# AI4quantum/twisteRL

Hardware: AMD Instinct MI355X
Metric: env-steps/s (whole node) Puzzle-15 PPO rollout (higher is better)
Workload: dtype f32; 1 GPU; Puzzle-15 PPO rollout + GAE + merge: 262144 envs/GPU, difficulty 128 (<= 257 records/episode), twists {identity, transpose}, BasicPolicy 256->512->256->4|1, gamma=lambda=0.995, torch-default-init weights seed 0; total_envs=262144, parallelism=episodes sharded x1

## Files before the change

### twisterl_amd/csrc/tw_engine.hpp

```cpp
#pragma once
#include <type_traits>
#include "tw_common.hpp"
#include "tw_engine_generic.hpp"
#include <cstdlib>

namespace tw {

typedef float f32x16 __attribute__((ext_vector_type(16)));
typedef float f32x4 __attribute__((ext_vector_type(4)));
typedef float f32x2 __attribute__((ext_vector_type(2)));
typedef __attribute__((address_space(3))) const float lds_cfloat;

constexpr int EPW = 32;


__device__ __forceinline__ float relu1(float x)
{
    float y;
    asm("v_max_f32 %0, 0, %1\n\ts_nop 1" : "=v"(y) : "v"(x));
    return y;
}
__device__ __forceinline__ float relu_lim(float x, float lim)
{
    float y;
    asm("v_max_f32 %0, %1, %2\n\ts_nop 1" : "=v"(y) : "s"(lim), "v"(x));
    return y;
}

__device__ __forceinline__ f32x2 pk_add(f32x2 a, f32x2 b)
{
    f32x2 r;
    r[0] = a[0] + b[0]; r[1] = a[1] + b[1];
    return r;
}

__device__ __forceinline__ float relu_lim_v(float x, float lim)
{
    float y;
    asm("v_max_f32 %0, %1, %2" : "=v"(y) : "s"(lim), "v"(x));
    return y;
}

__device__ __forceinline__ int gumbel_argmax4_halves(const float l[4], const u32x4 w, bool upper)
{
// ... 21 lines not shown

template <int NT>
__host__ __device__ inline size_t engine3_lds_floats(int obs_size)
{
    return (size_t)3 * R3_KC * Tiles<NT>::NQ * 128 + (size_t)3 * R3_TSLOT + (size_t)NT * 32 * 10 + 8 +
           (size_t)MAX_LDS_PERMS * ((obs_size + 3) / 4 + 1) + (size_t)NT * 32 * 5;
}

template <int NT, int NC, int NW_ = 8>
struct Engine3 {
    static constexpr int NW = NW_, KC = R3_KC, THREADS = 64 * NW_, EPB = NW * EPW, LSTR = R3_LSTR;
    static constexpr int NQ     = Tiles<NT>::NQ;
    static constexpr int WSLOT  = KC * NQ * 128;
    static constexpr int WPIECE = WSLOT / 256;
    static constexpr int TPIECE = ((NC * NC + 2) * R3_LSTR * 4 + 1023) / 1024;
    static_assert(TPIECE * 256 <= R3_TSLOT, "table chunk larger than its slot");
    static constexpr int NPIECE = WPIECE + TPIECE;
    static constexpr int NOPS   = (NPIECE + NW - 1) / NW;
    static constexpr int M      = 4 * NT;
    static constexpr bool SPLIT = false;

    __host__ __device__ static size_t lds_floats(int obs_size) { return engine3_lds_floats<NT>(obs_size); }
    __host__ __device__ static size_t lds_floats(const PolicyDev &p) { return lds_floats(p.obs_size); }
    __device__ __forceinline__ bool primary() const { return true; }
    __device__ __forceinline__ int  ep_lane() const { return wave * EPW + j; }
    __device__ __forceinline__ bool owns_lane() const { return true; }

    PolicyDev pol;
    int tid, lane, wave, j, h;
    uint32_t voff;
    int bias_row, zero_row, n_chunks;
    float emb_lim, common_lim;
    float *lds_w, *lds_t, *lds_b1, *lds_wh, *lds_bh, *lds_wn;
    const uint8_t *perm_obs, *perm_act;

    static_assert(WPIECE % NW == 0, "W1 pieces per chunk must be a multiple of the wave count");
    const uint8_t *dsrc_w, *dsrc_t;
    uint32_t ddst_w, ddst_t;
    __device__ __forceinline__ void stream_op(int chunk, int slot, int op)
    {
        if (NW * op < WPIECE) {
            const uint8_t *src = dsrc_w + (size_t)chunk * (WSLOT * 4) + (size_t)op * (NW * 1024);
            const uint32_t dst = ddst_w + (uint32_t)slot * (WSLOT * 4) + (uint32_t)op * (NW * 1024);
            TW_GLDS16(voff, dst, src);
        } else {
            const int T0 = NW * op - WPIECE;
            uint32_t tp = (uint32_t)wave + (uint32_t)T0;
            if (T0 + NW - 1 >= TPIECE) tp = tp < (uint32_t)TPIECE ? tp : (uint32_t)TPIECE - 1u;
            const uint8_t *src = dsrc_t + (size_t)chunk * (R3_TSLOT * 4) + (size_t)tp * 1024;
            const uint32_t dst = ddst_t + (uint32_t)slot * (R3_TSLOT * 4) + tp * 1024u;
            TW_GLDS16(voff, dst, src);
        }
    }

    __device__ __forceinline__ void begin1(const PolicyDev &p, float *lds)
    {
        pol = p;
        tid  = threadIdx.x;
        lane = tid & 63;
        wave = __builtin_amdgcn_readfirstlane(tid >> 6);
        j = lane & 31; h = lane >> 5;
        voff = (uint32_t)lane * 16u;
        bias_row = pol.obs_size; zero_row = pol.obs_size + 1;
        n_chunks = pol.emb / KC;
        emb_lim = pol.emb_relu ? 0.0f : -__builtin_inff();
        common_lim = pol.common_relu ? 0.0f : -__builtin_inff();
        lds_w  = lds;
        lds_t  = lds + 3 * WSLOT;
        lds_b1 = lds_t + 3 * R3_TSLOT;
        lds_wh = lds_b1 + NT * 32;
        lds_bh = lds_wh + NT * 32 * 9;
        dsrc_w = reinterpret_cast<const uint8_t *>(pol.w1p) + (size_t)wave * 1024;
        dsrc_t = reinterpret_cast<const uint8_t *>(pol.t_img16);
        ddst_w = __builtin_amdgcn_readfirstlane((unsigned)(uintptr_t)(__attribute__((address_space(3))) float *)lds_w) + (uint32_t)wave * 1024u;
        ddst_t = __builtin_amdgcn_readfirstlane((unsigned)(uintptr_t)(__attribute__((address_space(3))) float *)lds_t);
        for (int i = tid; i < NT * 32; i += THREADS) lds_b1[(i & 1) * (NT * 16) + (i >> 1)] = pol.b1[i];
        for (int i = tid; i < NT * 32 * 8; i += THREADS) {
            const int n = i >> 3, c = i & 7;
            lds_wh[(c * 2 + (n & 1)) * (NT * 16) + (n >> 1)] = pol.wh8[i];
        }
        for (int i = tid; i < NT * 32; i += THREADS) lds_wh[8 * 2 * (NT * 16) + i] = 0.0f;
        if (tid < 8) lds_bh[tid] = pol.bh8[tid];
        lds_wn = lds_bh + 8 + MAX_LDS_PERMS * ((pol.obs_size + 3) / 4 + 1);
        for (int i = tid; i < NT * 32 * 5; i += THREADS) {
            const int c = i / (NT * 32), n = i - c * (NT * 32);
            lds_wn[i] = pol.wh8[n * 8 + c];
        }
        perm_obs = pol.obs_perms; perm_act = pol.act_perms;
        if (pol.n_perms > 0 && pol.n_perms <= MAX_LDS_PERMS) {
            uint8_t *po = reinterpret_cast<uint8_t *>(lds_bh + 8);
            uint8_t *pa = po + MAX_LDS_PERMS * ((pol.obs_size + 3) / 4) * 4;
            for (int i = tid; i < pol.n_perms * pol.obs_size; i += THREADS) po[i] = pol.obs_perms[i];
            for (int i = tid; i < pol.n_perms * 4; i += THREADS) pa[i] = pol.act_perms[i];
            perm_obs = po; perm_act = pa;
        }
#pragma unroll
        for (int op = 0; op < NOPS; ++op) { stream_op(0, 0, op); stream_op(n_chunks > 1 ? 1 : 0, 1, op); }
    }
    __device__ __forceinline__ void begin2() { asm volatile("s_waitcnt vmcnt(0)" ::: "memory"); }
    __device__ __forceinline__ void end() { asm volatile("s_waitcnt vmcnt(0)" ::: "memory"); }

    __device__ __forceinline__ void rows_of(uint64_t board, int n_cells, int perm, int (&rowoff)[NC]) const
    {
#pragma unroll
        for (int i = 0; i < NC; ++i) {
            int row = zero_row;
            if (i < n_cells) {
                const int id = i * n_cells + (int)nib(board, i);
                row = perm >= 0 ? (int)perm_obs[perm * pol.obs_size + id] : id;
            }
            rowoff[i] = row * LSTR + h * (KC / 2);
        }
    }

    __device__ __forceinline__ void act_perm(int perm, float (&lg)[4]) const
    {
        if (perm < 0) return;
        const float l0 = lg[0], l1 = lg[1], l2 = lg[2], l3 = lg[3];
#pragma unroll
        for (int i = 0; i < 4; ++i) {
            const int src = perm_act[perm * 4 + i];
            lg[i] = src == 0 ? l0 : (src == 1 ? l1 : (src == 2 ? l2 : l3));
        }
    }

    __device__ __forceinline__ void finish_b(f32x4 &b) const
    {
        float x0 = b[0], x1 = b[1], x2 = b[2], x3 = b[3];
        asm("v_max_f32 %0, %4, %0\n\tv_max_f32 %1, %4, %1\n\tv_max_f32 %2, %4, %2\n\tv_max_f32 %3, %4, %3"
            : "+v"(x0), "+v"(x1), "+v"(x2), "+v"(x3) : "s"(emb_lim));
        b[0] = x0; b[1] = x1; b[2] = x2; b[3] = x3;
    }

    template <bool HAVE_NEXT_GATHER, bool LAST, bool CROSS>
    __device__ __forceinline__ void group(f32x16 (&acc)[NT], f32x4 (&aw)[NQ], const f32x4 bq, const float *w_base, int kp0,
                                          const float *wn_base, lds_cfloat *const (&ga)[NC + 1], int goff, f32x4 &bnext,
                                          int s_chunk, int s_slot, int op0, int op1)
    {
        constexpr int LAT = M >= 16 ? 4 : 1;
        auto rd_slot  = [](int q) constexpr { return M >= 16 ? (q * (M - 6)) / (NC + 1) : 0; };
        auto add_slot = [&](int q) constexpr { int v = rd_slot(q) + LAT; return v > M - 1 ? M - 1 : v; };
        f32x4 rd[NC + 1];
        f32x2 nlo, nhi;
#pragma unroll
        for (int m = 0; m < M; ++m) {
            const int u = m / NT, r = m % NT;
            acc[r] = __builtin_amdgcn_mfma_f32_32x32x2f32(aw[r / 4][r % 4], bq[u], acc[r], 0, 0, 0);
            __builtin_amdgcn_sched_barrier(0);
            if (r % 4 == 3 || r == NT - 1) {
                if (u < 3 || !LAST) aw[r / 4] = *reinterpret_cast<const f32x4 *>(w_base + ((kp0 + u + 1) * 2 * NQ + r / 4) * 128);
                else if (CROSS) aw[r / 4] = *reinterpret_cast<const f32x4 *>(wn_base + (r / 4) * 128);
            }
            {
                if constexpr (NW == 8) {
// ... 508 lines not shown
        this->tid = threadIdx.x; this->lane = this->tid & 63; this->wave = __builtin_amdgcn_readfirstlane(this->tid >> 6);
        this->j = this->lane & 15; this->h = this->lane >> 4;
        this->n_chunks = this->pol.emb / KC;
        np = (this->n_chunks + 1) / 2;
        n2 = (np + 1) / 2 * 2;
        __builtin_amdgcn_s_barrier();
    }
    __device__ __forceinline__ void idle_forward() const
    {
        for (int i = 0; i < n2 + 3; ++i) __builtin_amdgcn_s_barrier();
    }
    template <int SLOT, int OP = 0>
    __device__ __forceinline__ void stream_pair() const
    {
        if constexpr (OP < NOPS) { stream<SLOT, OP>(); stream_pair<SLOT, OP + 1>(); }
    }
    __device__ __forceinline__ int real_pair(int v) const { return v < np ? v : (v < n2 ? 0 : v - n2); }
    __device__ __forceinline__ void set_pointers()
    {
        stp  = this->dsrc_t + (size_t)real_pair(sv) * (2 * R3_TSLOT * 4);
        aoff = real_pair(av) * (2 * WSLOT);
    }
    __device__ __forceinline__ void advance()
    {
        ++sv; ++av; stp += 2 * R3_TSLOT * 4; aoff += 2 * WSLOT;
        if (sv == np || sv == n2) stp = this->dsrc_t;
        if (av == np || av == n2) aoff = 0;
        if (sv == n2) sv = 0;
        if (av == n2) av = 0;
    }

    __device__ __forceinline__ void rows_of(uint64_t board, int n_cells, int perm, int (&rowoff)[NC]) const
    {
#pragma unroll
        for (int i = 0; i < NC; ++i) {
            int row = this->zero_row;
            if (i < n_cells) {
                const int id = i * n_cells + (int)nib(board, i);
                row = perm >= 0 ? (int)this->perm_obs[perm * this->pol.obs_size + id] : id;
            }
            rowoff[i] = row * R3_LSTR;
        }
    }

    template <bool EB = false>
    __device__ __forceinline__ void forward(const int (&rowoff)[NC], float (&lg)[4], float &value)
    {
        typedef __attribute__((address_space(3))) const f32x4 lds_cf4;
        const int jj = this->j, kq = this->h, wave = this->wave;
        f32x4v acc[TPW];
#pragma unroll
        for (int t = 0; t < TPW; ++t) acc[t] = f32x4v{0.0f, 0.0f, 0.0f, 0.0f};

        lds_cfloat *gb = (lds_cfloat *)tbase + ((kq & 1) * 8 + 2 * wave + (kq >> 1));
        lds_cfloat *ga[NC + 1];
        ga[0] = gb + this->bias_row * R3_LSTR;
#pragma unroll
        for (int c = 0; c < NC; ++c) ga[c + 1] = gb + rowoff[c];

        float *xb = lds_x + 256;
        float gr[2][NC + 1];
        auto gather_finish = [&](int buf) {
#pragma unroll
            for (int hf = 0; hf < 2; ++hf) {
                float sm = gr[hf][0];
#pragma unroll
                for (int c = 1; c <= NC; ++c) sm = sm + gr[hf][c];
                xb[(buf * 64 + this->lane) * 8 + hf * 4 + wave] = relu_lim_v(sm, this->emb_lim);
            }
        };

        int par = 0;
        auto step = [&](auto pc, int p) {
            constexpr int P = decltype(pc)::value, Q = P ^ 1;
            constexpr int M = 8 * TPW;
// ... 102 lines not shown
```

### twisterl_amd/csrc/tw_engine16.hpp

```cpp
#pragma once
#include "tw_engine.hpp"

#include <type_traits>

namespace tw {

typedef _Float16 h16x8 __attribute__((ext_vector_type(8)));
typedef _Float16 h16x2 __attribute__((ext_vector_type(2)));
typedef __attribute__((address_space(3))) const uint8_t lds_cu8;

constexpr int E16_MAXP   = 4;
constexpr int E16_MAX_KT = 32;

template <int NHT, int NC>
__host__ __device__ constexpr size_t engine16_lds_bytes()
{
    return 160 + (size_t)(E16_MAXP + 1) * (16 + 256) + 32 + (size_t)2 * (E16_MAXP + 1) * 256 + 64 + (size_t)NHT * 128 + (size_t)E16_MAX_KT * 128 +
           (size_t)NHT * 2048 + (size_t)NC * 1024 + (size_t)3 * ((NC + 2 * NHT + 3) / 4) * 4096;
}

template <int NHT, int NC>
struct Engine16 {
    static constexpr int NW = 4, THREADS = 256, EPB = 256, D = 3;
    static constexpr int SP     = NC + 2 * NHT;
    static constexpr int NOPS   = (SP + NW - 1) / NW;
    static constexpr int SBYTES = NOPS * NW * 1024;
    static constexpr float OUT_SCALE = 1.0f;
    static constexpr bool SPLIT_RANGE = false;
    static constexpr uint32_t O_OH = 0, O_SRC = 160, O_VMAP = O_SRC + (E16_MAXP + 1) * 16, O_ACT = O_VMAP + (E16_MAXP + 1) * 256,
                              O_OHB = O_ACT + 32, O_BH = O_OHB + 2 * (E16_MAXP + 1) * 256, O_B1 = O_BH + 64, O_EBIAS = O_B1 + NHT * 128, O_HEAD = O_EBIAS + E16_MAX_KT * 128,
                              O_T0 = O_HEAD + NHT * 2048, O_RING = O_T0 + NC * 1024;
    static_assert(O_RING + 3 * SBYTES == engine16_lds_bytes<NHT, NC>(), "LDS map");

    struct Pipe { h16x8 a[D], x0[D], x1[D]; f32x16 eb; };
    struct OneHots { uint32_t a0[NC], a1[NC]; };

    PolicyDev pol;
    int tid, lane, wave, j, hh, n_kt, rp;
    TW_STAMP_VARS(st[8] = {});
    uint8_t *lg_;
    uint32_t lds_u32, voff;
    lds_cu8 *L;
// ... 34 lines not shown
        for (int i = tid; i < np1 * 16; i += THREADS) lds[O_SRC + i] = pol.srcmap16[i];
        for (int i = tid; i < np1 * 256; i += THREADS) lds[O_VMAP + i] = pol.vmap16[i];
        for (int i = tid; i < 2 * np1 * 256; i += THREADS) {
            const int h2 = i / (np1 * 256), r = i - h2 * (np1 * 256);
            const uint32_t pos = (uint32_t)pol.vmap16[r] ^ ((uint32_t)h2 << 3);
            lds[O_OHB + h2 * ((E16_MAXP + 1) * 256) + r] = (uint8_t)((pos < 8u ? pos : 8u) * 16u);
        }
        if (tid < 4) lds[O_ACT + tid] = (uint8_t)tid;
        for (int i = tid; i < pol.n_perms * 4; i += THREADS) lds[O_ACT + 4 + i] = pol.act_perms[i];
        for (int i = tid; i < n_kt * 32; i += THREADS) reinterpret_cast<float *>(lds + O_EBIAS)[i] = pol.ebias16[i];
#pragma unroll
        for (int op = 0; op < NOPS; ++op) { stream_op(stage_ptr(0), slot_m0(0), op); stream_op(stage_ptr(n_kt > 1 ? 1 : 0), slot_m0(1), op); }
        rp = 0;
    }
    __device__ __forceinline__ void begin2() { asm volatile("s_waitcnt vmcnt(0)" ::: "memory"); }
    __device__ __forceinline__ void end() { asm volatile("s_waitcnt vmcnt(0)" ::: "memory"); }

    __device__ __forceinline__ void onehots(uint64_t board, int perm, uint32_t (&w)[NC]) const
    {
        static_assert(O_OH == 0, "the byte table holds LDS addresses");
        const int pi = perm + 1;
        typedef uint32_t u32v4 __attribute__((ext_vector_type(4)));
        const u32v4 sr = *(const __attribute__((address_space(3))) u32v4 *)(L + O_SRC + pi * 16);
        const uint32_t srw[4] = {sr[0], sr[1], sr[2], sr[3]};
        const uint32_t tb = O_OHB + (uint32_t)(hh * (E16_MAXP + 1) + pi) * 256u;
#pragma unroll
        for (int c = 0; c < NC; ++c) {
            const uint32_t src = (srw[c >> 2] >> (8 * (c & 3))) & 0xffu;
            const uint32_t v   = nib(board, (int)src);
            w[c] = L[tb + c * 16 + v];
        }
    }

    __device__ __forceinline__ void act_perm(int perm, float (&lg)[4]) const
    {
        typedef __attribute__((address_space(3))) const uint32_t lu1;
        const uint32_t ap = *(const lu1 *)(L + O_ACT + (perm + 1) * 4);
        const float l0 = lg[0], l1 = lg[1], l2 = lg[2], l3 = lg[3];
#pragma unroll
        for (int i = 0; i < 4; ++i) {
            const uint32_t src = (ap >> (8 * i)) & 0xffu;
            lg[i] = src == 0 ? l0 : (src == 1 ? l1 : (src == 2 ? l2 : l3));
        }
    }

    __device__ __forceinline__ f32x16 ld16(uint32_t off) const
    {
        typedef __attribute__((address_space(3))) const f32x4 lf4;
        const lf4 *p = (const lf4 *)(L + off);
        const f32x4 a = p[0], b = p[1], c = p[2], d = p[3];
        f32x16 r;
#pragma unroll
        for (int i = 0; i < 4; ++i) { r[i] = a[i]; r[4 + i] = b[i]; r[8 + i] = c[i]; r[12 + i] = d[i]; }
        return r;
    }
    __device__ __forceinline__ h16x8 ld8(uint32_t off) const
    {
        return *(const __attribute__((address_space(3))) h16x8 *)(L + off);
    }
    static __device__ __forceinline__ void mfma_v(f32x16 &d, const h16x8 a, const h16x8 b, bool first, const f32x16 &c0)
    {
        if (first) asm volatile("v_mfma_f32_32x32x16_f16 %0, %1, %2, %3" : "=&v"(d) : "v"(a), "v"(b), "v"(c0));
        else       asm volatile("v_mfma_f32_32x32x16_f16 %0, %1, %2, %0" : "+v"(d) : "v"(a), "v"(b));
    }
    template <bool BIAS>
    static __device__ __forceinline__ void cvt_unit(const f32x16 &e, const f32x16 &bias, int m, int q, h16x2 lim, h16x8 &dst)
// ... 208 lines not shown
```

### twisterl_amd/csrc/tw_engine16x2.hpp

```cpp
#pragma once
#include "tw_engine16.hpp"

#include <utility>

namespace tw {

template <int NHT, int NC>
__host__ __device__ constexpr int engineS_pieces() { return (NC + 2 * NHT > 4 * NHT) ? NC + 2 * NHT : 4 * NHT; }
template <int NHT, int NC>
__host__ __device__ constexpr size_t engineS_lds_bytes()
{
    return 160 + (size_t)(E16_MAXP + 1) * (16 + 256) + 32 + (size_t)2 * (E16_MAXP + 1) * 256 + 64 + (size_t)NHT * 128 +
           (size_t)E16_MAX_KT * 128 + (size_t)2 * NC * 1024 + (size_t)3 * ((engineS_pieces<NHT, NC>() + 3) / 4) * 4096;
}

template <int NHT, int NC>
struct EngineS {
    static constexpr int NW = 4, THREADS = 256, EPB = 256, D = 3;
    static constexpr int NM0    = 2 * NHT;
    static constexpr int SP     = engineS_pieces<NHT, NC>();
    static constexpr int NOPS   = (SP + NW - 1) / NW;
    static constexpr int SBYTES = NOPS * NW * 1024;
    static constexpr float OUT_SCALE = 1.0f / 4096.0f;
    static constexpr bool SPLIT_RANGE = true;
// ... 47 lines not shown
        for (int i = tid; i < np1 * 16; i += THREADS) lds[O_SRC + i] = pol.srcmap16[i];
        for (int i = tid; i < np1 * 256; i += THREADS) lds[O_VMAP + i] = pol.vmap16[i];
        for (int i = tid; i < 2 * np1 * 256; i += THREADS) {
            const int h2 = i / (np1 * 256), r = i - h2 * (np1 * 256);
            const uint32_t pos = (uint32_t)pol.vmap16[r] ^ ((uint32_t)h2 << 3);
            lds[O_OHB + h2 * ((E16_MAXP + 1) * 256) + r] = (uint8_t)((pos < 8u ? pos : 8u) * 16u);
        }
        if (tid < 4) lds[O_ACT + tid] = (uint8_t)tid;
        for (int i = tid; i < pol.n_perms * 4; i += THREADS) lds[O_ACT + 4 + i] = pol.act_perms[i];
        for (int i = tid; i < n_kt * 32; i += THREADS) reinterpret_cast<float *>(lds + O_EBIAS)[i] = pol.ebias16[i] * 16.0f;
#pragma unroll
        for (int op = 0; op < NOPS; ++op) { stream_op(stage_ptr(0), slot_m0(0), op); stream_op(stage_ptr(1), slot_m0(1), op); }
        rp = 0;
    }
    __device__ __forceinline__ void begin2() { asm volatile("s_waitcnt vmcnt(0)" ::: "memory"); }
    __device__ __forceinline__ void end() { asm volatile("s_waitcnt vmcnt(0)" ::: "memory"); }

    __device__ __forceinline__ void onehots(uint64_t board, int perm, uint32_t (&w)[(NC + 3) / 4]) const
    {
        static_assert(O_OH == 0, "the byte table holds LDS addresses");
        const int pi = perm + 1;
        typedef uint32_t u32v4 __attribute__((ext_vector_type(4)));
        const u32v4 sr = *(const __attribute__((address_space(3))) u32v4 *)(L + O_SRC + pi * 16);
        const uint32_t srw[4] = {sr[0], sr[1], sr[2], sr[3]};
        const uint32_t tb = O_OHB + (uint32_t)(hh * (E16_MAXP + 1) + pi) * 256u;
#pragma unroll
        for (int q = 0; q < (NC + 3) / 4; ++q) w[q] = 0u;
#pragma unroll
        for (int c = 0; c < NC; ++c) {
            const uint32_t src = (srw[c >> 2] >> (8 * (c & 3))) & 0xffu;
            w[c >> 2] |= (uint32_t)L[tb + c * 16 + nib(board, (int)src)] << (8 * (c & 3));
        }
    }
    __device__ __forceinline__ h16x8 ldoh(const uint32_t (&w)[(NC + 3) / 4], int c) const
    {
        return ld8(O_OH + ((w[c >> 2] >> (8 * (c & 3))) & 0xffu));
    }
    __device__ __forceinline__ void act_perm(int perm, float (&lg)[4]) const
    {
        typedef __attribute__((address_space(3))) const uint32_t lu1;
        const uint32_t ap = *(const lu1 *)(L + O_ACT + (perm + 1) * 4);
        const float l0 = lg[0], l1 = lg[1], l2 = lg[2], l3 = lg[3];
#pragma unroll
        for (int i = 0; i < 4; ++i) {
            const uint32_t src = (ap >> (8 * i)) & 0xffu;
            lg[i] = src == 0 ? l0 : (src == 1 ? l1 : (src == 2 ? l2 : l3));
        }
    }
    __device__ __forceinline__ f32x16 ld16(uint32_t off) const
    {
        typedef __attribute__((address_space(3))) const f32x4 lf4;
        const lf4 *p = (const lf4 *)(L + off);
        const f32x4 a = p[0], b = p[1], c = p[2], d = p[3];
        f32x16 r;
#pragma unroll
        for (int i = 0; i < 4; ++i) { r[i] = a[i]; r[4 + i] = b[i]; r[8 + i] = c[i]; r[12 + i] = d[i]; }
        return r;
    }
    __device__ __forceinline__ h16x8 ld8(uint32_t off) const { return *(const __attribute__((address_space(3))) h16x8 *)(L + off); }
    static __device__ __forceinline__ void mfma_v(f32x16 &d, const h16x8 a, const h16x8 b, bool first, const f32x16 &c0)
    {
        if (first) asm volatile("v_mfma_f32_32x32x16_f16 %0, %1, %2, %3" : "=&v"(d) : "v"(a), "v"(b), "v"(c0));
        else       asm volatile("v_mfma_f32_32x32x16_f16 %0, %1, %2, %0" : "+v"(d) : "v"(a), "v"(b));
    }
    static __device__ __forceinline__ void split_unit(const f32x16 &e, int m, int q, float lim, h16x8 &hi, h16x8 &lo)
    {
// ... 228 lines not shown
```

### twisterl_amd/csrc/tw_rollout.hip

```cpp
#include "tw_engine.hpp"

#include <cstdlib>
#include <cstring>

namespace tw {

__global__ void __launch_bounds__(256) init_boards_kernel(const PuzzleConsts env, uint64_t seed, uint64_t episode_offset, uint64_t n, uint64_t *out, uint4 *entries)
{
    const uint64_t i = (uint64_t)blockIdx.x * 256 + threadIdx.x;
    if (i >= n) return;
    PuzzleLane st;
    puzzle_reset(st, env, seed, episode_offset + i);
    if (out) out[i] = st.board;
    if (entries) entries[i] = make_uint4((uint32_t)st.board, (uint32_t)(st.board >> 32), (uint32_t)i, 0u);
}

int launch_init_boards(const PuzzleConsts &env, uint64_t seed, uint64_t episode_offset, uint64_t n, uint64_t *out, hipStream_t s, uint4 *entries)
{
    if (n == 0) return TW_OK;
    hipLaunchKernelGGL(init_boards_kernel, dim3((unsigned)((n + 255) / 256)), dim3(256), 0, s, env, seed, episode_offset, n, out, entries);
    TW_HIP(hipGetLastError());
    return TW_OK;
}

// ... 115 lines not shown
TW_STAMP_ARRAY(g_gen_stamps, 8);

template <int NT, int NC, int NW = 8, bool PERSIST = false>
__global__ void __launch_bounds__((Geom<NT, NC, NW>::WAVES * 64), ((NW == 8 || NW == -65) ? 2 : 1)) rollout_f32_kernel(const RolloutArgs a)
{
    using Eng = typename Geom<NT, NC, NW>::Eng;
    extern __shared__ __attribute__((aligned(16))) float lds[];
    Eng eng;
    eng.begin1(a.pol, lds);

    const PuzzleConsts env = a.env;
    const int j = eng.j, h = eng.h;
    const uint64_t e_first = (uint64_t)blockIdx.x * Eng::EPB + (uint64_t)eng.ep_lane();
    const bool valid  = e_first < a.num_episodes;
    const bool writer = h == 0 && eng.primary();
    uint32_t e_local = (uint32_t)e_first;
    uint64_t board = env.ident; int depth = 0;
    if (valid) {
        if constexpr (PERSIST) {
            const uint4 ib = a.init_boards[e_local];
            e_local = ib.z; board = ((uint64_t)ib.y << 32) | ib.x; depth = env.depth0;
        }
        else { PuzzleLane s0; puzzle_reset(s0, env, a.seed, a.episode_offset + e_first); board = s0.board; depth = s0.depth; }
    }

    bool     alive = valid;
    bool     more  = PERSIST;
    int      t = 0;

    eng.begin2();
    TW_STAMP(q_loop);
    TW_STAMP_VARS(n_fwd = 0);

    while (__syncthreads_or(alive ? 1 : 0)) {
        TW_STAMP_COUNT(n_fwd, 1);
        int perm = -1;
        if (eng.pol.n_perms > 0) {
            const u32x4 w = rng_draw(a.seed, a.episode_offset + (uint64_t)e_local, (uint32_t)t, STREAM_PERM);
            perm = (int)u32_below(w.x, (uint32_t)eng.pol.n_perms);
        }
        int rowoff[NC];
        eng.rows_of(board, env.n_cells, perm, rowoff);

        float lg[4]; float value;
        eng.forward(rowoff, lg, value);

        PuzzleLane st; st.board = board; st.depth = depth;
        { const int z = blank_cell(board); st.zx = z % env.width; st.zy = z / env.width; }
        eng.act_perm(perm, lg);
        const uint32_t mb = puzzle_maskbits(st, env);
#pragma unroll
        for (int i = 0; i < 4; ++i) lg[i] = ((mb >> i) & 1u) ? lg[i] : -1e10f;
        const float rew = puzzle_reward(st, env);
        const u32x4 gw = rng_draw(a.seed, a.episode_offset + (uint64_t)e_local, (uint32_t)t, STREAM_GUMBEL);
        int action;
        if constexpr (NW == 8) action = gumbel_argmax4_halves(lg, gw, h != 0);
        else action = gumbel_argmax4(lg, gw);
        if (alive) {
            if (writer) {
                const uint64_t rec = (uint64_t)e_local * (uint64_t)a.out.t_pad + (uint64_t)t;
                uint32_t obs_base[4], pk[4];
                obs_base_words(env.n_cells, obs_base);
                obs_bytes(board, obs_base, pk);
                store_rec(a.out.rec + rec, pk, lg, value, rew, action, perm);
            }
            if (puzzle_final(st, env)) {
                alive = false;
                if constexpr (PERSIST) { if (writer) a.out.ep_len[e_local] = (uint32_t)t + 1u; }
            } else { puzzle_step(st, env, action); board = st.board; depth = st.depth; ++t; }
        }
        if constexpr (PERSIST) {
            const bool want = !alive && more;
            unsigned got = 0xffffffffu;
            if (want && writer) got = atomicAdd(a.queue, 1u);
            if constexpr (Eng::SPLIT) {
                unsigned *bc = reinterpret_cast<unsigned *>(eng.lds_user);
                if (writer) bc[j] = got;
                __syncthreads();
                got = bc[j];
            } else got = (unsigned)__shfl((int)got, j, 64);
            if (want) {
                if ((uint64_t)got < a.num_episodes) {
                    const uint4 ib = a.init_boards[got];
                    e_local = ib.z; board = ((uint64_t)ib.y << 32) | ib.x; depth = env.depth0;
                    alive = true; t = 0;
                } else more = false;
            }
        }
    }
    if constexpr (!PERSIST) { if (valid && writer) a.out.ep_len[e_local] = (uint32_t)t + 1u; }
    eng.end();
    if constexpr (NW == -65)
        TW_STAMP_FLUSH(eng.lane == 0 && (eng.wave == 0 || eng.wave == 3), g_gen_stamps + (eng.wave ? 4 : 0), eng.stq[0], eng.stq[1], eng.stq[2], eng.stq[3]);
    if constexpr (NW == -16 || NW == -4) {
        TW_STAMP(q_end);
        TW_STAMP_FLUSH(eng.lane == 0 && eng.wave == 0, g_gen_stamps, eng.stq[0], eng.stq[1], eng.stq[2], eng.stq[3], eng.stq[4], n_fwd, q_end - q_loop);
    }
}

static uint64_t persist_blocks(int reserve_cus)
{
    const int cus = device_cus();
    const int r = reserve_cus < 0 ? 0 : (reserve_cus > cus - 1 ? cus - 1 : reserve_cus);
    return (uint64_t)(cus - r);
}

uint64_t rollout_f32_resident_episodes(int reserve_cus) { return persist_blocks(reserve_cus) * 8 * EPW; }

static uint64_t generic_groups_per_cu(const PolicyDev &pol, int n_cells)
{
    const size_t lds_bytes = (n_cells <= 4 ? EngineV<4>::lds_floats(pol) : (n_cells <= 9 ? EngineV<9>::lds_floats(pol) : EngineV<16>::lds_floats(pol))) * sizeof(float);
    return lds_bytes * 2 <= 159 * 1024 ? 2 : 1;
}
uint64_t rollout_generic_resident_episodes(const PolicyDev &pol, int n_cells, int reserve_cus) { return persist_blocks(reserve_cus) * generic_groups_per_cu(pol, n_cells) * 16; }

uint64_t f32_resident_episodes(uint64_t num_episodes, int hidden, bool selfplay, int reserve_cus)
{
    const uint64_t full = rollout_f32_resident_episodes(reserve_cus), small = full / 8;
// ... 103 lines not shown
```

### twisterl_amd/csrc/tw_rollout16.hip

```cpp
#include "tw_engine16x2.hpp"

#include <cstdio>
#include <cstdlib>

namespace tw {

TW_STAMP_ARRAY(g_stamps16, 8);

template <class Eng, int NC, bool PERSIST = false>
__global__ void __launch_bounds__(256, 1) rollout_f16_kernel(const RolloutArgs a)
{
    extern __shared__ __attribute__((aligned(16))) uint8_t lds16[];
    TW_STAMP(t_kernel0);
    Eng eng;
    eng.begin1(a.pol, lds16);

    const PuzzleConsts env = a.env;
    const int j = eng.j, hh = eng.hh;
    uint64_t   e_own  = (uint64_t)blockIdx.x * Eng::EPB + (uint64_t)(eng.wave * 64 + hh * 32 + j);
    const bool v_own  = e_own < a.num_episodes;
    uint64_t   eg_own = a.episode_offset + e_own;

    auto from_board = [&](uint64_t b) {
        PuzzleLane s; s.board = b;
        const int z = blank_cell(b);
        s.zx = z % env.width; s.zy = z / env.width; s.depth = env.depth0;
        return s;
    };
    PuzzleLane own;
    own.board = env.ident; own.zx = 0; own.zy = 0; own.depth = 0;
    if (v_own) {
        if constexpr (PERSIST) {
            const uint4 ib = a.init_boards[e_own];
            e_own = ib.z; eg_own = a.episode_offset + e_own;
            own = from_board(((uint64_t)ib.y << 32) | ib.x);
        } else puzzle_reset(own, env, a.seed, eg_own);
    }
    PuzzleLane st0, st1;
    {
        PuzzleLane oth;
        oth.board = ((uint64_t)(uint32_t)__shfl_xor((int)(uint32_t)(own.board >> 32), 32, 64) << 32) |
                    (uint64_t)(uint32_t)__shfl_xor((int)(uint32_t)own.board, 32, 64);
        oth.zx = __shfl_xor(own.zx, 32, 64); oth.zy = __shfl_xor(own.zy, 32, 64); oth.depth = __shfl_xor(own.depth, 32, 64);
        st0 = hh ? oth : own; st1 = hh ? own : oth;
    }
    const bool v_oth = __shfl_xor(v_own ? 1 : 0, 32, 64) != 0;
    bool alive0 = hh ? v_oth : v_own, alive1 = hh ? v_own : v_oth;
    int      t = 0;
    uint32_t len_own = 0;
    float    out_max = 0.0f;
    uint64_t rec_base = e_own * (uint64_t)a.out.t_pad;
    bool     more = PERSIST;

    uint32_t obs_base[4];
    obs_base_words(env.n_cells, obs_base);
    float bh[5];
#pragma unroll
    for (int i = 0; i < 5; ++i) bh[i] = a.pol.bh16[i];

    eng.begin2();
    TW_STAMP_VARS(t_prev = __builtin_readcyclecounter());
    while (__syncthreads_or((alive0 || alive1) ? 1 : 0)) {
        TW_STAMP(t_top);
        TW_STAMP_ADD(eng.st[7], t_prev, t_top);
        int perm_own = -1;
        if (eng.pol.n_perms > 0) {
            const u32x4 w = rng_draw(a.seed, eg_own, (uint32_t)t, STREAM_PERM);
            perm_own = (int)u32_below(w.x, (uint32_t)eng.pol.n_perms);
        }
        const int perm_oth = __shfl_xor(perm_own, 32, 64);
        const int perm0 = hh ? perm_oth : perm_own, perm1 = hh ? perm_own : perm_oth;
        typename Eng::OneHots oh;
        eng.onehots(st0.board, perm0, oh.a0);
        eng.onehots(st1.board, perm1, oh.a1);

        TW_STAMP_USE(oh.a0[0]); TW_STAMP_USE(oh.a1[0]);
        TW_STAMP(t_fw);
        TW_STAMP_ADD(eng.st[0], t_top, t_fw);
        f32x16 out0, out1;
        eng.forward(oh, out0, out1);
        TW_STAMP(t_po);

        float lg[4];
#pragma unroll
        for (int i = 0; i < 4; ++i) lg[i] = (hh ? out1[i] : out0[i]) * Eng::OUT_SCALE + bh[i];
        const float value = (hh ? out1[4] : out0[4]) * Eng::OUT_SCALE + bh[4];
        if constexpr (Eng::SPLIT_RANGE) {
#pragma unroll
            for (int i = 0; i < 4; ++i) out_max = __builtin_elementwise_maximum(out_max, __builtin_fabsf(lg[i]));
            out_max = __builtin_elementwise_maximum(out_max, __builtin_fabsf(value));
        }
        PuzzleLane mine;
        mine.board = hh ? st1.board : st0.board; mine.zx = hh ? st1.zx : st0.zx; mine.zy = hh ? st1.zy : st0.zy;
        mine.depth = hh ? st1.depth : st0.depth;
        eng.act_perm(perm_own, lg);
        const uint32_t mb = puzzle_maskbits(mine, env);
#pragma unroll
        for (int i = 0; i < 4; ++i) lg[i] = ((mb >> i) & 1u) ? lg[i] : -1e10f;
        const float rew = puzzle_reward(mine, env);
        const u32x4 gw = rng_draw(a.seed, eg_own, (uint32_t)t, STREAM_GUMBEL);
        const int act_own = gumbel_argmax4(lg, gw);
        const bool alive_own = hh ? alive1 : alive0;
        if (alive_own) {
            uint32_t pk[4];
            obs_bytes(mine.board, obs_base, pk);
            store_rec(a.out.rec + rec_base + (uint64_t)t, pk, lg, value, rew, act_own, perm_own);
        }
        const int act_oth = __shfl_xor(act_own, 32, 64);
        const int act0 = hh ? act_oth : act_own, act1 = hh ? act_own : act_oth;
        {
            const bool fin0 = puzzle_final(st0, env), fin1 = puzzle_final(st1, env);
            PuzzleLane n0 = st0, n1 = st1;
            puzzle_step(n0, env, act0); puzzle_step(n1, env, act1);
            const bool go0 = alive0 && !fin0, go1 = alive1 && !fin1;
            st0.board = go0 ? n0.board : st0.board; st0.zx = go0 ? n0.zx : st0.zx; st0.zy = go0 ? n0.zy : st0.zy; st0.depth = go0 ? n0.depth : st0.depth;
            st1.board = go1 ? n1.board : st1.board; st1.zx = go1 ? n1.zx : st1.zx; st1.zy = go1 ? n1.zy : st1.zy; st1.depth = go1 ? n1.depth : st1.depth;
            const bool died_own = hh ? (alive1 && fin1) : (alive0 && fin0);
            len_own = died_own ? (uint32_t)t + 1u : len_own;
            alive0 = go0; alive1 = go1;
            if constexpr (PERSIST) { if (died_own) a.out.ep_len[e_own] = len_own; }
        }
        ++t;
        if constexpr (PERSIST) {
            const bool idle_own = !(hh ? alive1 : alive0);
            unsigned got = 0xffffffffu;
            if (idle_own && more) got = atomicAdd(a.queue, 1u);
            const bool took = (uint64_t)got < a.num_episodes;
            more = more && !(idle_own && !took);
            uint64_t nb = 0;
            if (took) { const uint4 ib = a.init_boards[got]; e_own = ib.z; eg_own = a.episode_offset + e_own; rec_base = e_own * (uint64_t)a.out.t_pad; t = 0; nb = ((uint64_t)ib.y << 32) | ib.x; }
            const bool took_oth = __shfl_xor(took ? 1 : 0, 32, 64) != 0;
            const uint64_t nb_oth = ((uint64_t)(uint32_t)__shfl_xor((int)(uint32_t)(nb >> 32), 32, 64) << 32) |
                                    (uint64_t)(uint32_t)__shfl_xor((int)(uint32_t)nb, 32, 64);
            const PuzzleLane n_own = from_board(nb), n_oth = from_board(nb_oth);
            const bool t0 = hh ? took_oth : took, t1 = hh ? took : took_oth;
            const PuzzleLane &n0 = hh ? n_oth : n_own, &n1 = hh ? n_own : n_oth;
            if (t0) { st0 = n0; alive0 = true; }
            if (t1) { st1 = n1; alive1 = true; }
        }
        TW_RESTAMP(t_prev);
        TW_STAMP_ADD(eng.st[6], t_po, t_prev);
    }
    TW_STAMP(t_kernel1);
    TW_STAMP_FLUSH(eng.lane == 0, g_stamps16, eng.st[0], eng.st[1], eng.st[2], t_kernel1 - t_kernel0,
                   eng.st[4], eng.st[5], eng.st[6], eng.st[7]);
    if constexpr (!PERSIST) { if (v_own) a.out.ep_len[e_own] = len_own; }
    if constexpr (Eng::SPLIT_RANGE) {
        if (!(out_max <= 3.0e38f)) atomicOr(a.range_flag, 1u);
    }
    eng.end();
}

template <class Eng, int NC, bool PERSIST>
static int launch16p(const RolloutArgs &a, hipStream_t s, uint32_t *blocks, uint32_t *threads, size_t lds_bytes)
{
    const uint64_t nb = PERSIST ? rollout_f32_resident_episodes(a.reserve_cus) / Eng::EPB : (a.num_episodes + Eng::EPB - 1) / Eng::EPB;
    if (nb == 0 || nb > 0x7fffffffull) { set_error("rollout16: bad episode count %llu", (unsigned long long)a.num_episodes); return TW_ERR_INVALID; }
    if (lds_bytes > 159 * 1024) { set_error("rollout16: %zu bytes of LDS needed, 159 KiB available", lds_bytes); return TW_ERR_UNSUPPORTED; }
    if (int rc = ensure_dynamic_lds(reinterpret_cast<const void *>(&rollout_f16_kernel<Eng, NC, PERSIST>), lds_bytes)) return rc;
    TW_STAMPS_CLEAR(g_stamps16);
    hipLaunchKernelGGL((rollout_f16_kernel<Eng, NC, PERSIST>), dim3((unsigned)nb), dim3(Eng::THREADS), lds_bytes, s, a);
    TW_HIP(hipGetLastError());
    TW_STAMPS_REPORT(g_stamps16, s, h, {
        const double nw = (double)nb * 4.0;
        fprintf(stderr, "[stamps16] per wave (cycles x100MHz ticks): pre %.0f prologue %.0f stage-body %.0f vmcnt %.0f stage-barrier %.0f heads %.0f post %.0f step-barrier %.0f\n",
                h[0] / nw, h[1] / nw, h[2] / nw, h[3] / nw, h[4] / nw, h[5] / nw, h[6] / nw, h[7] / nw);
    });
    if (blocks) *blocks = (uint32_t)nb;
    if (threads) *threads = Eng::THREADS;
    return TW_OK;
}

template <class Eng, int NC>
static int launch16(const RolloutArgs &a, hipStream_t s, uint32_t *blocks, uint32_t *threads, size_t lds_bytes)
{
    if (a.queue && a.init_boards && a.num_episodes > rollout_f32_resident_episodes(a.reserve_cus)) return launch16p<Eng, NC, true>(a, s, blocks, threads, lds_bytes);
    return launch16p<Eng, NC, false>(a, s, blocks, threads, lds_bytes);
}

// ... 53 lines not shown
```

Before: 487.6 million env-steps/s.

## Simplify per-lane rollout state and cut register pressure in rollout kernels

The f16 rollout kernel drops the duplicated two-episode state per lane (st0/st1 with shuffles). Each lane now keeps only its own board, and one-hot addresses are built via permlane32_swap. Depth and blank position are recomputed from the board, and the head biases are read from LDS each step. The f32 engine always indexes permutation tables through LDS address-space pointers with clamped, branch-free lookups. The f32 rollout merges the perm draw and the Gumbel draw into one RNG call split across wave halves. The aim is fewer VGPRs, shuffles and RNG evaluations, at the cost of extra recomputation and changed RNG stream pairing in the NW==8 path.

```diff
diff --git a/twisterl_amd/csrc/tw_engine.hpp b/twisterl_amd/csrc/tw_engine.hpp
--- a/twisterl_amd/csrc/tw_engine.hpp
+++ b/twisterl_amd/csrc/tw_engine.hpp
@@ -10,6 +10,7 @@
 typedef float f32x4 __attribute__((ext_vector_type(4)));
 typedef float f32x2 __attribute__((ext_vector_type(2)));
 typedef __attribute__((address_space(3))) const float lds_cfloat;
+typedef __attribute__((address_space(3))) const uint8_t lds_cu8;
 
 constexpr int EPW = 32;
 
@@ -97,7 +98,8 @@
     int bias_row, zero_row, n_chunks;
     float emb_lim, common_lim;
     float *lds_w, *lds_t, *lds_b1, *lds_wh, *lds_bh, *lds_wn;
-    const uint8_t *perm_obs, *perm_act;
+    lds_cu8 *perm_obs, *perm_act;
+    bool perms_lds;
 
     static_assert(WPIECE % NW == 0, "W1 pieces per chunk must be a multiple of the wave count");
     const uint8_t *dsrc_w, *dsrc_t;
@@ -151,13 +153,15 @@
             const int c = i / (NT * 32), n = i - c * (NT * 32);
             lds_wn[i] = pol.wh8[n * 8 + c];
         }
-        perm_obs = pol.obs_perms; perm_act = pol.act_perms;
-        if (pol.n_perms > 0 && pol.n_perms <= MAX_LDS_PERMS) {
+        {
             uint8_t *po = reinterpret_cast<uint8_t *>(lds_bh + 8);
             uint8_t *pa = po + MAX_LDS_PERMS * ((pol.obs_size + 3) / 4) * 4;
-            for (int i = tid; i < pol.n_perms * pol.obs_size; i += THREADS) po[i] = pol.obs_perms[i];
-            for (int i = tid; i < pol.n_perms * 4; i += THREADS) pa[i] = pol.act_perms[i];
-            perm_obs = po; perm_act = pa;
+            perms_lds = pol.n_perms <= MAX_LDS_PERMS;
+            if (perms_lds) {
+                for (int i = tid; i < pol.n_perms * pol.obs_size; i += THREADS) po[i] = pol.obs_perms[i];
+                for (int i = tid; i < pol.n_perms * 4; i += THREADS) pa[i] = pol.act_perms[i];
+            }
+            perm_obs = (lds_cu8 *)po; perm_act = (lds_cu8 *)pa;
         }
 #pragma unroll
         for (int op = 0; op < NOPS; ++op) { stream_op(0, 0, op); stream_op(n_chunks > 1 ? 1 : 0, 1, op); }
@@ -165,26 +169,59 @@
     __device__ __forceinline__ void begin2() { asm volatile("s_waitcnt vmcnt(0)" ::: "memory"); }
     __device__ __forceinline__ void end() { asm volatile("s_waitcnt vmcnt(0)" ::: "memory"); }
 
+    __device__ __forceinline__ void twisted_rows(uint64_t board, int n_cells, int perm, int (&row)[NC]) const
+    {
+        typedef const __attribute__((address_space(1))) uint8_t glb_cu8;
+        const uint32_t pbase = (uint32_t)(perm >= 0 ? perm : 0) * (uint32_t)pol.obs_size;
+        const uint32_t nn = (uint32_t)(n_cells * n_cells);
+        uint32_t id[NC], at[NC], tw[NC];
+#pragma unroll
+        for (int i = 0; i < NC; ++i) {
+            id[i] = (uint32_t)(i * n_cells) + (uint32_t)nib(board, i);
+            at[i] = pbase + (id[i] < nn ? id[i] : nn - 1u);
+        }
+        if (__builtin_expect(perms_lds, 1)) {
+#pragma unroll
+            for (int i = 0; i < NC; ++i) tw[i] = perm_obs[at[i]];
+        } else {
+            glb_cu8 *g = (glb_cu8 *)pol.obs_perms;
+#pragma unroll
+            for (int i = 0; i < NC; ++i) tw[i] = g[at[i]];
+#pragma unroll
+            for (int i = 0; i < NC; ++i) asm volatile("" : "+v"(tw[i]));
+        }
+#pragma unroll
+        for (int i = 0; i < NC; ++i) {
+            const uint32_t r = perm >= 0 ? tw[i] : id[i];
+            row[i] = (int)(id[i] < nn ? r : (uint32_t)zero_row);
+        }
+    }
+
     __device__ __forceinline__ void rows_of(uint64_t board, int n_cells, int perm, int (&rowoff)[NC]) const
     {
-#pragma unroll
-        for (int i = 0; i < NC; ++i) {
-            int row = zero_row;
-            if (i < n_cells) {
-                const int id = i * n_cells + (int)nib(board, i);
-                row = perm >= 0 ? (int)perm_obs[perm * pol.obs_size + id] : id;
-            }
-            rowoff[i] = row * LSTR + h * (KC / 2);
-        }
+        int row[NC];
+        twisted_rows(board, n_cells, perm, row);
+#pragma unroll
+        for (int i = 0; i < NC; ++i) rowoff[i] = row[i] * LSTR + h * (KC / 2);
     }
 
     __device__ __forceinline__ void act_perm(int perm, float (&lg)[4]) const
     {
-        if (perm < 0) return;
+        typedef const __attribute__((address_space(1))) uint8_t glb_cu8;
+        typedef __attribute__((address_space(3))) const uint32_t lds_cu32;
+        const uint32_t at = (uint32_t)(perm >= 0 ? perm : 0) * 4u;
+        uint32_t ap;
+        if (perms_lds) ap = *(lds_cu32 *)(perm_act + at);
+        else {
+            glb_cu8 *g = (glb_cu8 *)pol.act_perms + at;
+            const uint32_t b0 = g[0], b1 = g[1], b2 = g[2], b3 = g[3];
+            ap = b0 | (b1 << 8) | (b2 << 16) | (b3 << 24);
+        }
+        ap = perm >= 0 ? ap : 0x03020100u;
         const float l0 = lg[0], l1 = lg[1], l2 = lg[2], l3 = lg[3];
 #pragma unroll
         for (int i = 0; i < 4; ++i) {
-            const int src = perm_act[perm * 4 + i];
+            const uint32_t src = (ap >> (8 * i)) & 0xffu;
             lg[i] = src == 0 ? l0 : (src == 1 ? l1 : (src == 2 ? l2 : l3));
         }
     }
@@ -759,15 +796,10 @@
 
     __device__ __forceinline__ void rows_of(uint64_t board, int n_cells, int perm, int (&rowoff)[NC]) const
     {
-#pragma unroll
-        for (int i = 0; i < NC; ++i) {
-            int row = this->zero_row;
-            if (i < n_cells) {
-                const int id = i * n_cells + (int)nib(board, i);
-                row = perm >= 0 ? (int)this->perm_obs[perm * this->pol.obs_size + id] : id;
-            }
-            rowoff[i] = row * R3_LSTR;
-        }
+        int row[NC];
+        this->twisted_rows(board, n_cells, perm, row);
+#pragma unroll
+        for (int i = 0; i < NC; ++i) rowoff[i] = row[i] * R3_LSTR;
     }
 
     template <bool EB = false>
diff --git a/twisterl_amd/csrc/tw_engine16.hpp b/twisterl_amd/csrc/tw_engine16.hpp
--- a/twisterl_amd/csrc/tw_engine16.hpp
+++ b/twisterl_amd/csrc/tw_engine16.hpp
@@ -7,7 +7,6 @@
 
 typedef _Float16 h16x8 __attribute__((ext_vector_type(8)));
 typedef _Float16 h16x2 __attribute__((ext_vector_type(2)));
-typedef __attribute__((address_space(3))) const uint8_t lds_cu8;
 
 constexpr int E16_MAXP   = 4;
 constexpr int E16_MAX_KT = 32;
@@ -108,6 +107,45 @@
         }
     }
 
+    __device__ __forceinline__ void twisted_values(uint64_t board, int perm, uint32_t (&pk)[(NC + 3) / 4]) const
+    {
+        const int pi = perm + 1;
+        typedef uint32_t u32v4 __attribute__((ext_vector_type(4)));
+        const u32v4 sr = *(const __attribute__((address_space(3))) u32v4 *)(L + O_SRC + pi * 16);
+        const uint32_t srw[4] = {sr[0], sr[1], sr[2], sr[3]};
+        const uint32_t tb = O_VMAP + (uint32_t)pi * 256u;
+        uint32_t v[NC];
+#pragma unroll
+        for (int c = 0; c < NC; ++c) {
+            const uint32_t src = (srw[c >> 2] >> (8 * (c & 3))) & 0xffu;
+            v[c] = L[tb + c * 16 + nib(board, (int)src)];
+        }
+#pragma unroll
+        for (int q = 0; q < (NC + 3) / 4; ++q) pk[q] = 0u;
+#pragma unroll
+        for (int c = 0; c < NC; ++c) pk[c >> 2] |= v[c] << (8 * (c & 3));
+    }
+    __device__ __forceinline__ uint32_t onehot_addr4(uint32_t vals) const
+    {
+        static_assert(O_OH == 0, "the bytes are LDS addresses");
+        const uint32_t p = vals ^ (hh ? 0x08080808u : 0u);
+        const uint32_t m = p & 0x08080808u;
+        return (p & ~(m - (m >> 3))) << 4;
+    }
+    __device__ __forceinline__ void onehots_own(uint64_t board, int perm, OneHots &oh) const
+    {
+        uint32_t pk[(NC + 3) / 4];
+        twisted_values(board, perm, pk);
+#pragma unroll
+        for (int q = 0; q < (NC + 3) / 4; ++q) {
+            const auto sw = __builtin_amdgcn_permlane32_swap(pk[q], pk[q], false, false);
+            const uint32_t a0 = onehot_addr4(sw[0]), a1 = onehot_addr4(sw[1]);
+#pragma unroll
+            for (int b = 0; b < 4; ++b)
+                if (4 * q + b < NC) { oh.a0[4 * q + b] = (a0 >> (8 * b)) & 0xffu; oh.a1[4 * q + b] = (a1 >> (8 * b)) & 0xffu; }
+        }
+    }
+
     __device__ __forceinline__ void act_perm(int perm, float (&lg)[4]) const
     {
         typedef __attribute__((address_space(3))) const uint32_t lu1;
diff --git a/twisterl_amd/csrc/tw_engine16x2.hpp b/twisterl_amd/csrc/tw_engine16x2.hpp
--- a/twisterl_amd/csrc/tw_engine16x2.hpp
+++ b/twisterl_amd/csrc/tw_engine16x2.hpp
@@ -103,6 +103,35 @@
             w[c >> 2] |= (uint32_t)L[tb + c * 16 + nib(board, (int)src)] << (8 * (c & 3));
         }
     }
+    __device__ __forceinline__ void onehots_own(uint64_t board, int perm, OneHots &oh) const
+    {
+        static_assert(O_OH == 0, "the bytes are LDS addresses");
+        const int pi = perm + 1;
+        typedef uint32_t u32v4 __attribute__((ext_vector_type(4)));
+        const u32v4 sr = *(const __attribute__((address_space(3))) u32v4 *)(L + O_SRC + pi * 16);
+        const uint32_t srw[4] = {sr[0], sr[1], sr[2], sr[3]};
+        const uint32_t tb = O_VMAP + (uint32_t)pi * 256u;
+        uint32_t v[NC], pk[(NC + 3) / 4];
+#pragma unroll
+        for (int c = 0; c < NC; ++c) {
+            const uint32_t src = (srw[c >> 2] >> (8 * (c & 3))) & 0xffu;
+            v[c] = L[tb + c * 16 + nib(board, (int)src)];
+        }
+#pragma unroll
+        for (int q = 0; q < (NC + 3) / 4; ++q) pk[q] = 0u;
+#pragma unroll
+        for (int c = 0; c < NC; ++c) pk[c >> 2] |= v[c] << (8 * (c & 3));
+        auto addr4 = [&](uint32_t vals) {
+            const uint32_t p = vals ^ (hh ? 0x08080808u : 0u);
+            const uint32_t m = p & 0x08080808u;
+            return (p & ~(m - (m >> 3))) << 4;
+        };
+#pragma unroll
+        for (int q = 0; q < (NC + 3) / 4; ++q) {
+            const auto sw = __builtin_amdgcn_permlane32_swap(pk[q], pk[q], false, false);
+            oh.a0[q] = addr4(sw[0]); oh.a1[q] = addr4(sw[1]);
+        }
+    }
     __device__ __forceinline__ h16x8 ldoh(const uint32_t (&w)[(NC + 3) / 4], int c) const
     {
         return ld8(O_OH + ((w[c >> 2] >> (8 * (c & 3))) & 0xffu));
diff --git a/twisterl_amd/csrc/tw_rollout.hip b/twisterl_amd/csrc/tw_rollout.hip
--- a/twisterl_amd/csrc/tw_rollout.hip
+++ b/twisterl_amd/csrc/tw_rollout.hip
@@ -171,18 +171,31 @@
     TW_STAMP(q_loop);
     TW_STAMP_VARS(n_fwd = 0);
 
+    constexpr bool ONE_DRAW = NW == 8;
+    auto seed_here = [&]() {
+        uint32_t lo = (uint32_t)a.seed, hi = (uint32_t)(a.seed >> 32);
+        asm volatile("" : "+s"(lo), "+s"(hi));
+        return ((uint64_t)hi << 32) | lo;
+    };
+    auto draw_perm = [&](uint32_t e, int tt) {
+        const u32x4 w = rng_draw(seed_here(), a.episode_offset + (uint64_t)e, (uint32_t)tt, STREAM_PERM);
+        return (int)u32_below(w.x, (uint32_t)eng.pol.n_perms);
+    };
+    int perm_next = -1;
+    if constexpr (ONE_DRAW) { if (eng.pol.n_perms > 0) perm_next = draw_perm(e_local, 0); }
+
     while (__syncthreads_or(alive ? 1 : 0)) {
         TW_STAMP_COUNT(n_fwd, 1);
+        if constexpr (!PERSIST) asm volatile("" : "+v"(e_local));
         int perm = -1;
-        if (eng.pol.n_perms > 0) {
-            const u32x4 w = rng_draw(a.seed, a.episode_offset + (uint64_t)e_local, (uint32_t)t, STREAM_PERM);
-            perm = (int)u32_below(w.x, (uint32_t)eng.pol.n_perms);
-        }
+        if constexpr (ONE_DRAW) perm = perm_next;
+        else if (eng.pol.n_perms > 0) perm = draw_perm(e_local, t);
         int rowoff[NC];
         eng.rows_of(board, env.n_cells, perm, rowoff);
 
         float lg[4]; float value;
         eng.forward(rowoff, lg, value);
+        if constexpr (!PERSIST) asm volatile("" : "+v"(e_local));
 
         PuzzleLane st; st.board = board; st.depth = depth;
         { const int z = blank_cell(board); st.zx = z % env.width; st.zy = z / env.width; }
@@ -191,10 +204,17 @@
 #pragma unroll
         for (int i = 0; i < 4; ++i) lg[i] = ((mb >> i) & 1u) ? lg[i] : -1e10f;
         const float rew = puzzle_reward(st, env);
-        const u32x4 gw = rng_draw(a.seed, a.episode_offset + (uint64_t)e_local, (uint32_t)t, STREAM_GUMBEL);
         int action;
-        if constexpr (NW == 8) action = gumbel_argmax4_halves(lg, gw, h != 0);
-        else action = gumbel_argmax4(lg, gw);
+        if constexpr (ONE_DRAW) {
+            const u32x4 w = rng_draw(seed_here(), a.episode_offset + (uint64_t)e_local, (uint32_t)(h ? t : t + 1), h ? STREAM_GUMBEL : STREAM_PERM);
+            const auto sx = __builtin_amdgcn_permlane32_swap(w.x, w.x, false, false);
+            const auto sy = __builtin_amdgcn_permlane32_swap(w.y, w.y, false, false);
+            perm_next = eng.pol.n_perms > 0 ? (int)u32_below(sx[0], (uint32_t)eng.pol.n_perms) : -1;
+            action = gumbel_argmax4_halves(lg, u32x4{sx[1], sy[1], w.z, w.w}, h != 0);
+        } else {
+            const u32x4 gw = rng_draw(seed_here(), a.episode_offset + (uint64_t)e_local, (uint32_t)t, STREAM_GUMBEL);
+            action = gumbel_argmax4(lg, gw);
+        }
         if (alive) {
             if (writer) {
                 const uint64_t rec = (uint64_t)e_local * (uint64_t)a.out.t_pad + (uint64_t)t;
@@ -223,6 +243,7 @@
                     const uint4 ib = a.init_boards[got];
                     e_local = ib.z; board = ((uint64_t)ib.y << 32) | ib.x; depth = env.depth0;
                     alive = true; t = 0;
+                    if constexpr (ONE_DRAW) { if (eng.pol.n_perms > 0) perm_next = draw_perm(e_local, 0); }
                 } else more = false;
             }
         }
diff --git a/twisterl_amd/csrc/tw_rollout16.hip b/twisterl_amd/csrc/tw_rollout16.hip
--- a/twisterl_amd/csrc/tw_rollout16.hip
+++ b/twisterl_amd/csrc/tw_rollout16.hip
@@ -16,63 +16,45 @@
     eng.begin1(a.pol, lds16);
 
     const PuzzleConsts env = a.env;
-    const int j = eng.j, hh = eng.hh;
-    uint64_t   e_own  = (uint64_t)blockIdx.x * Eng::EPB + (uint64_t)(eng.wave * 64 + hh * 32 + j);
-    const bool v_own  = e_own < a.num_episodes;
-    uint64_t   eg_own = a.episode_offset + e_own;
-
-    auto from_board = [&](uint64_t b) {
-        PuzzleLane s; s.board = b;
-        const int z = blank_cell(b);
-        s.zx = z % env.width; s.zy = z / env.width; s.depth = env.depth0;
-        return s;
+    const int hh = eng.hh;
+    uint32_t   e_q = 0;
+    auto first_episode = [&]() -> uint64_t {
+        uint32_t e_lane = (uint32_t)(eng.wave * 64 + eng.lane);
+        asm volatile("" : "+v"(e_lane));
+        return (uint64_t)blockIdx.x * Eng::EPB + e_lane;
     };
-    PuzzleLane own;
-    own.board = env.ident; own.zx = 0; own.zy = 0; own.depth = 0;
-    if (v_own) {
-        if constexpr (PERSIST) {
-            const uint4 ib = a.init_boards[e_own];
-            e_own = ib.z; eg_own = a.episode_offset + e_own;
-            own = from_board(((uint64_t)ib.y << 32) | ib.x);
-        } else puzzle_reset(own, env, a.seed, eg_own);
-    }
-    PuzzleLane st0, st1;
-    {
-        PuzzleLane oth;
-        oth.board = ((uint64_t)(uint32_t)__shfl_xor((int)(uint32_t)(own.board >> 32), 32, 64) << 32) |
-                    (uint64_t)(uint32_t)__shfl_xor((int)(uint32_t)own.board, 32, 64);
-        oth.zx = __shfl_xor(own.zx, 32, 64); oth.zy = __shfl_xor(own.zy, 32, 64); oth.depth = __shfl_xor(own.depth, 32, 64);
-        st0 = hh ? oth : own; st1 = hh ? own : oth;
-    }
-    const bool v_oth = __shfl_xor(v_own ? 1 : 0, 32, 64) != 0;
-    bool alive0 = hh ? v_oth : v_own, alive1 = hh ? v_own : v_oth;
+    const bool v_own  = first_episode() < a.num_episodes;
+    auto episode = [&]() -> uint64_t {
+        if constexpr (PERSIST) return (uint64_t)e_q;
+        else return first_episode();
+    };
+
+    uint64_t board = env.ident;
+    if constexpr (PERSIST) {
+        if (v_own) {
+            const uint4 ib = a.init_boards[first_episode()];
+            e_q = ib.z; board = ((uint64_t)ib.y << 32) | ib.x;
+        }
+    } else {
+        PuzzleLane s0; puzzle_reset(s0, env, a.seed, a.episode_offset + episode()); board = s0.board;
+    }
+    bool     alive = v_own;
     int      t = 0;
-    uint32_t len_own = 0;
     float    out_max = 0.0f;
-    uint64_t rec_base = e_own * (uint64_t)a.out.t_pad;
     bool     more = PERSIST;
-
-    uint32_t obs_base[4];
-    obs_base_words(env.n_cells, obs_base);
-    float bh[5];
-#pragma unroll
-    for (int i = 0; i < 5; ++i) bh[i] = a.pol.bh16[i];
 
     eng.begin2();
     TW_STAMP_VARS(t_prev = __builtin_readcyclecounter());
-    while (__syncthreads_or((alive0 || alive1) ? 1 : 0)) {
+    while (__syncthreads_or(alive ? 1 : 0)) {
         TW_STAMP(t_top);
         TW_STAMP_ADD(eng.st[7], t_prev, t_top);
         int perm_own = -1;
         if (eng.pol.n_perms > 0) {
-            const u32x4 w = rng_draw(a.seed, eg_own, (uint32_t)t, STREAM_PERM);
+            const u32x4 w = rng_draw(a.seed, a.episode_offset + episode(), (uint32_t)t, STREAM_PERM);
             perm_own = (int)u32_below(w.x, (uint32_t)eng.pol.n_perms);
         }
-        const int perm_oth = __shfl_xor(perm_own, 32, 64);
-        const int perm0 = hh ? perm_oth : perm_own, perm1 = hh ? perm_own : perm_oth;
         typename Eng::OneHots oh;
-        eng.onehots(st0.board, perm0, oh.a0);
-        eng.onehots(st1.board, perm1, oh.a1);
+        eng.onehots_own(board, perm_own, oh);
 
         TW_STAMP_USE(oh.a0[0]); TW_STAMP_USE(oh.a1[0]);
         TW_STAMP(t_fw);
@@ -81,6 +63,13 @@
         eng.forward(oh, out0, out1);
         TW_STAMP(t_po);
 
+        float bh[5];
+        {
+            typedef __attribute__((address_space(3))) const float lds_cf;
+            const f32x4 b4 = *(__attribute__((address_space(3))) const f32x4 *)(eng.L + Eng::O_BH);
+            bh[0] = b4[0]; bh[1] = b4[1]; bh[2] = b4[2]; bh[3] = b4[3];
+            bh[4] = *(lds_cf *)(eng.L + Eng::O_BH + 16);
+        }
         float lg[4];
 #pragma unroll
         for (int i = 0; i < 4; ++i) lg[i] = (hh ? out1[i] : out0[i]) * Eng::OUT_SCALE + bh[i];
@@ -90,9 +79,10 @@
             for (int i = 0; i < 4; ++i) out_max = __builtin_elementwise_maximum(out_max, __builtin_fabsf(lg[i]));
             out_max = __builtin_elementwise_maximum(out_max, __builtin_fabsf(value));
         }
+        const uint64_t e_own = episode(), eg_own = a.episode_offset + e_own;
         PuzzleLane mine;
-        mine.board = hh ? st1.board : st0.board; mine.zx = hh ? st1.zx : st0.zx; mine.zy = hh ? st1.zy : st0.zy;
-        mine.depth = hh ? st1.depth : st0.depth;
+        mine.board = board; mine.depth = env.depth0 > t ? env.depth0 - t : 0;
+        { const int z = blank_cell(board); mine.zx = z % env.width; mine.zy = z / env.width; }
         eng.act_perm(perm_own, lg);
         const uint32_t mb = puzzle_maskbits(mine, env);
 #pragma unroll
@@ -100,43 +90,30 @@
         const float rew = puzzle_reward(mine, env);
         const u32x4 gw = rng_draw(a.seed, eg_own, (uint32_t)t, STREAM_GUMBEL);
         const int act_own = gumbel_argmax4(lg, gw);
-        const bool alive_own = hh ? alive1 : alive0;
-        if (alive_own) {
-            uint32_t pk[4];
-            obs_bytes(mine.board, obs_base, pk);
-            store_rec(a.out.rec + rec_base + (uint64_t)t, pk, lg, value, rew, act_own, perm_own);
-        }
-        const int act_oth = __shfl_xor(act_own, 32, 64);
-        const int act0 = hh ? act_oth : act_own, act1 = hh ? act_own : act_oth;
+        if (alive) {
+            uint32_t obs_base[4], pk[4];
+            obs_base_words(env.n_cells, obs_base);
+            obs_bytes(board, obs_base, pk);
+            store_rec(a.out.rec + e_own * (uint64_t)a.out.t_pad + (uint64_t)t, pk, lg, value, rew, act_own, perm_own);
+        }
         {
-            const bool fin0 = puzzle_final(st0, env), fin1 = puzzle_final(st1, env);
-            PuzzleLane n0 = st0, n1 = st1;
-            puzzle_step(n0, env, act0); puzzle_step(n1, env, act1);
-            const bool go0 = alive0 && !fin0, go1 = alive1 && !fin1;
-            st0.board = go0 ? n0.board : st0.board; st0.zx = go0 ? n0.zx : st0.zx; st0.zy = go0 ? n0.zy : st0.zy; st0.depth = go0 ? n0.depth : st0.depth;
-            st1.board = go1 ? n1.board : st1.board; st1.zx = go1 ? n1.zx : st1.zx; st1.zy = go1 ? n1.zy : st1.zy; st1.depth = go1 ? n1.depth : st1.depth;
-            const bool died_own = hh ? (alive1 && fin1) : (alive0 && fin0);
-            len_own = died_own ? (uint32_t)t + 1u : len_own;
-            alive0 = go0; alive1 = go1;
-            if constexpr (PERSIST) { if (died_own) a.out.ep_len[e_own] = len_own; }
+            const bool fin = puzzle_final(mine, env);
+            puzzle_step(mine, env, act_own);
+            const bool go = alive && !fin;
+            board = go ? mine.board : board;
+            if (alive && fin) a.out.ep_len[e_own] = (uint32_t)t + 1u;
+            alive = go;
         }
         ++t;
         if constexpr (PERSIST) {
-            const bool idle_own = !(hh ? alive1 : alive0);
             unsigned got = 0xffffffffu;
-            if (idle_own && more) got = atomicAdd(a.queue, 1u);
+            if (!alive && more) got = atomicAdd(a.queue, 1u);
             const bool took = (uint64_t)got < a.num_episodes;
-            more = more && !(idle_own && !took);
-            uint64_t nb = 0;
-            if (took) { const uint4 ib = a.init_boards[got]; e_own = ib.z; eg_own = a.episode_offset + e_own; rec_base = e_own * (uint64_t)a.out.t_pad; t = 0; nb = ((uint64_t)ib.y << 32) | ib.x; }
-            const bool took_oth = __shfl_xor(took ? 1 : 0, 32, 64) != 0;
-            const uint64_t nb_oth = ((uint64_t)(uint32_t)__shfl_xor((int)(uint32_t)(nb >> 32), 32, 64) << 32) |
-                                    (uint64_t)(uint32_t)__shfl_xor((int)(uint32_t)nb, 32, 64);
-            const PuzzleLane n_own = from_board(nb), n_oth = from_board(nb_oth);
-            const bool t0 = hh ? took_oth : took, t1 = hh ? took : took_oth;
-            const PuzzleLane &n0 = hh ? n_oth : n_own, &n1 = hh ? n_own : n_oth;
-            if (t0) { st0 = n0; alive0 = true; }
-            if (t1) { st1 = n1; alive1 = true; }
+            more = more && (alive || took);
+            if (took) {
+                const uint4 ib = a.init_boards[got];
+                e_q = ib.z; t = 0; board = ((uint64_t)ib.y << 32) | ib.x; alive = true;
+            }
         }
         TW_RESTAMP(t_prev);
         TW_STAMP_ADD(eng.st[6], t_po, t_prev);
@@ -144,7 +121,6 @@
     TW_STAMP(t_kernel1);
     TW_STAMP_FLUSH(eng.lane == 0, g_stamps16, eng.st[0], eng.st[1], eng.st[2], t_kernel1 - t_kernel0,
                    eng.st[4], eng.st[5], eng.st[6], eng.st[7]);
-    if constexpr (!PERSIST) { if (v_own) a.out.ep_len[e_own] = len_own; }
     if constexpr (Eng::SPLIT_RANGE) {
         if (!(out_max <= 3.0e38f)) atomicOr(a.range_flag, 1u);
     }
```

Measured after the change: 487.5 million env-steps/s (median of 3 runs). About the same (-0.0%).
